# DLR-RB/QUEASARS

Hardware: AMD Instinct MI355X
Metric: circuit-evals/sec (EVQE population) at n qubits; achieved HBM GB/s vs roofline (higher is better)
Workload: dtype f64; 1 GPU; 20-qubit EVQE population=64 per GPU, 4 layers, random Ising Hamiltonian (210 terms), fp64 (BASELINE.json configs[1]); n_qubits=20, population_per_gpu=64, layers=4, pauli_terms=210, parallelism=1 GPU

## Files before the change

include/qsv.h:

```cpp
#ifndef QSV_H
#define QSV_H

#include <stddef.h>
#include <stdint.h>

#ifdef __cplusplus
extern "C" {
#endif

typedef struct qsv_handle qsv_t;

enum { QSV_OP_ID = 0, QSV_OP_U = 1, QSV_OP_CU3 = 2 };
enum { QSV_F64 = 0, QSV_F32 = 1 };
enum { QSV_NO_CONTROL = 0xFF };

enum {
    QSV_OK = 0,
    QSV_E_ARG = -1,
    QSV_E_DEVICE = -2,
    QSV_E_STATE = -3,
    QSV_E_UNSUPPORTED = -4
};

typedef struct qsv_op {
// ... 227 lines not shown
int qsv_adjoint_describe(int n_qubits, int n_ops, const qsv_op* ops, int n_params, int n_wrt, const int32_t* wrt, int capacity_runs,
                         uint64_t* out_masks, int32_t* out_first_op, int32_t* out_last_op, int64_t* out_n_gates,
                         int32_t* out_tile_bits, int32_t* out_low_bits);
int qsv_adjoint_gradient_circuits(qsv_t* h, int n_evals, const int* circuit_ids, const int64_t* param_offsets, const double* params,
                                  const int64_t* wrt_offsets , const int32_t* wrt,
                                  double* out , double* out_values );
int qsv_adjoint_gradient_device(qsv_t* h, int n_evals, const int* circuit_ids, int width, const double* device_values, void* ready_event,
                                const int64_t* wrt_offsets, const int32_t* wrt, int out_width, double* device_out,
                                double* device_out_values );
typedef struct qsv_adjoint_stats_t {
    int64_t n_gates;
    int64_t n_runs;
    int64_t n_state_sweeps;
    int64_t scratch_bytes;
    int64_t n_allocations;
} qsv_adjoint_stats_t;
int qsv_adjoint_stats(const qsv_t* h, qsv_adjoint_stats_t* out);


int qsv_observables_create(qsv_t* h, int n_observables, const int64_t* term_offsets, const uint64_t* x_mask,
                           const uint64_t* z_mask, const double* coeff_re, const double* coeff_im, int* out_set_id);
int qsv_observables_destroy(qsv_t* h, int set_id);
int qsv_eval_observables(qsv_t* h, int set_id, int n_evals, const int* circuit_ids, const int64_t* param_offsets,
                         const double* params, double* out);


#define QSV_TABLE_SENTINEL 0x7FF8C0DEC0DE0001ull
int qsv_fitness_table_wait(const volatile uint64_t* own, int count, volatile int64_t* done, int stride, int world, int rank,
                           int64_t step, int budget_us);


int qsv_set_option(qsv_t* h, const char* name, int value);

long long qsv_replayed_pushes(const qsv_t* h);

int qsv_set_profiling(qsv_t* h, int enabled);
int qsv_get_profile(const qsv_t* h, qsv_profile* out);

int qsv_bench_gate(qsv_t* h, int target, int control, double theta, double phi, double lambda, int reps,
                   double* out_ms_per_sweep);

int qsv_bench_ops(qsv_t* h, int n_ops, const qsv_op* ops, int reps, double* out_ms_per_rep, int* out_n_passes);

int qsv_plan_build(int n_qubits, int dtype, int n_ops, const qsv_op* ops, const qsv_plan_config* cfg,
                   uint32_t* out_words, size_t capacity_words, size_t* n_words);

int qsv_split_describe(int n_qubits, int n_ops, const qsv_op* ops, int max_side, uint64_t* mask_a, qsv_op* ops_a,
                       int capacity_a, int* n_ops_a, qsv_op* ops_b, int capacity_b, int* n_ops_b);

#define QSV_SPLIT_MAX_KEYS 8
int qsv_split_describe_reduced(int n_qubits, int n_ops, const qsv_op* ops, int max_side, uint64_t* mask_a, qsv_op* ops_a,
                               int capacity_a, int* n_ops_a, qsv_op* ops_b, int capacity_b, int* n_ops_b,
                               uint32_t* simulated_keys, uint32_t* final_keys, int* key_bits, int* qubits);

const char* qsv_version(void);

#ifdef __cplusplus
}
#endif
#endif
```

queasars_amd/_lib.py:

```python

from __future__ import annotations

import ctypes as C
import os
import threading
from pathlib import Path

import numpy as np

from queasars_amd import _build

QSV_OK, QSV_E_ARG, QSV_E_DEVICE, QSV_E_STATE, QSV_E_UNSUPPORTED = 0, -1, -2, -3, -4
QSV_F64, QSV_F32 = 0, 1


class QsvOp(C.Structure):
    _fields_ = [
        ("kind", C.c_uint8),
        ("target", C.c_uint8),
        ("control", C.c_uint8),
        ("flags", C.c_uint8),
        ("p_theta", C.c_int32),
        ("p_phi", C.c_int32),
        ("p_lambda", C.c_int32),
# ... 224 lines not shown
    "qsv_statevector": (C.c_int, [_P, C.c_int, _P, C.c_int, _P]),
    "qsv_probabilities": (C.c_int, [_P, C.c_int, _P, C.c_int, _P]),
    "qsv_sample": (C.c_int, [_P, C.c_int, _P, C.c_int, C.c_int, C.c_uint64, _P]),
    "qsv_sample_batch": (C.c_int, [_P, C.c_int, _P, _P, _P, C.c_int, C.c_uint64, _P, _P]),
    "qsv_sample_cvar_batch": (C.c_int, [_P, C.c_int, _P, _P, _P, C.c_int, C.c_uint64, C.c_double, _P]),
    "qsv_exact_cvar_batch": (C.c_int, [_P, C.c_int, _P, _P, _P, C.c_double, _P]),
    "qsv_top_states": (C.c_int, [_P, C.c_int, _P, _P, _P, C.c_int, _P, _P, _P]),
    "qsv_cvar_device": (C.c_int, [_P, C.c_int, _P, C.c_int, _P, _P, C.c_int, C.c_uint64, C.c_double, _P, C.c_int, _P]),
    "qsv_value_cache_create": (C.c_int, [_P, C.c_int, C.c_int, _P]),
    "qsv_value_cache_destroy": (C.c_int, [_P, C.c_int]),
    "qsv_value_cache_clear": (C.c_int, [_P, C.c_int]),
    "qsv_value_cache_stats": (C.c_int, [_P, C.c_int, _P]),
    "qsv_sample_lookup": (C.c_int, [_P, C.c_int, C.c_int, _P, _P, _P, C.c_int, C.c_uint64, _P, _P]),
    "qsv_sample_lookup_finish": (C.c_int, [_P, C.c_int, C.c_int64, _P, C.c_double, _P, _P]),
    "qsv_gradient_describe": (C.c_int, [C.c_int, _P, C.c_int, _P]),
    "qsv_gradient_circuits": (C.c_int, [_P, C.c_int, _P, _P, _P, _P, _P, _P, _P]),
    "qsv_gradient_device": (C.c_int, [_P, C.c_int, _P, C.c_int, _P, _P, _P, _P, C.c_int, _P, _P]),
    "qsv_gradient_stats": (C.c_int, [_P, C.POINTER(QsvGradientStats)]),
    "qsv_gradient_plan_create": (C.c_int, [_P, C.c_int, _P, C.c_int, _P, _P, C.c_int, C.POINTER(C.c_int), C.POINTER(C.c_int64)]),
    "qsv_gradient_plan_run": (C.c_int, [_P, C.c_int, _P, _P, _P]),
    "qsv_gradient_plan_destroy": (C.c_int, [_P, C.c_int]),
    "qsv_gradient_plan_stats": (C.c_int, [_P, C.c_int, C.POINTER(QsvGradientPlanStats)]),
    "qsv_adjoint_describe": (C.c_int, [C.c_int, C.c_int, _P, C.c_int, C.c_int, _P, C.c_int, _P, _P, _P, C.POINTER(C.c_int64),
                                       C.POINTER(C.c_int32), C.POINTER(C.c_int32)]),
    "qsv_adjoint_gradient_circuits": (C.c_int, [_P, C.c_int, _P, _P, _P, _P, _P, _P, _P]),
    "qsv_adjoint_gradient_device": (C.c_int, [_P, C.c_int, _P, C.c_int, _P, _P, _P, _P, C.c_int, _P, _P]),
    "qsv_adjoint_stats": (C.c_int, [_P, C.POINTER(QsvAdjointStats)]),
    "qsv_observables_create": (C.c_int, [_P, C.c_int, _P, _P, _P, _P, _P, C.POINTER(C.c_int)]),
    "qsv_observables_destroy": (C.c_int, [_P, C.c_int]),
    "qsv_eval_observables": (C.c_int, [_P, C.c_int, C.c_int, _P, _P, _P, _P]),
    "qsv_set_option": (C.c_int, [_P, C.c_char_p, C.c_int]),
    "qsv_fitness_table_wait": (C.c_int, [C.c_void_p, C.c_int, C.c_void_p, C.c_int, C.c_int, C.c_int, C.c_int64, C.c_int]),
    "qsv_replayed_pushes": (C.c_longlong, [_P]),
    "qsv_set_profiling": (C.c_int, [_P, C.c_int]),
    "qsv_get_profile": (C.c_int, [_P, C.POINTER(QsvProfile)]),
    "qsv_bench_gate": (C.c_int, [_P, C.c_int, C.c_int, C.c_double, C.c_double, C.c_double, C.c_int, C.POINTER(C.c_double)]),
    "qsv_bench_ops": (C.c_int, [_P, C.c_int, _P, C.c_int, C.POINTER(C.c_double), C.POINTER(C.c_int)]),
    "qsv_split_describe": (
        C.c_int,
        [C.c_int, C.c_int, _P, C.c_int, C.POINTER(C.c_uint64), _P, C.c_int, C.POINTER(C.c_int), _P, C.c_int, C.POINTER(C.c_int)],
    ),
    "qsv_split_describe_reduced": (
        C.c_int,
        [C.c_int, C.c_int, _P, C.c_int, C.POINTER(C.c_uint64), _P, C.c_int, C.POINTER(C.c_int), _P, C.c_int, C.POINTER(C.c_int),
         _P, _P, _P, _P],
    ),
    "qsv_plan_build": (
        C.c_int,
        [C.c_int, C.c_int, C.c_int, _P, C.POINTER(QsvPlanConfig), _P, C.c_size_t, C.POINTER(C.c_size_t)],
    ),
}

_lock = threading.Lock()
_lib = None


class QsvLibraryError(RuntimeError):
    """libqsv is missing or could not be loaded.  There is deliberately no fallback."""


def library_path() -> Path:
    override = os.environ.get("QSV_LIBRARY")
    return Path(override) if override else _build.LIB_PATH


def load(build_if_missing: bool = True) -> C.CDLL:
# ... 36 lines not shown
```

queasars_amd/csrc/kernels.hip:

```cpp
#include "kernels.hpp"
#include "plan.hpp"

#include <hip/hip_runtime.h>

#include <type_traits>
#include <utility>

namespace qsv {

template <typename real>
struct alignas(2 * sizeof(real)) cx {
    real re, im;
};

#if defined(__HIP_DEVICE_COMPILE__)
#define QSV_CONST_AS __attribute__((address_space(4)))
#else
#define QSV_CONST_AS
#endif
using cu32p = const QSV_CONST_AS uint32_t*;
using cf64p = const QSV_CONST_AS double*;
template <typename T>
__device__ __forceinline__ const QSV_CONST_AS T* as_constant(const T* p) {
    return (const QSV_CONST_AS T*)(p);
// ... 3095 lines not shown
            out[0 * 64 + pi] = acc_one[e];
            out[1 * 64 + pi] = acc_d[e];
#pragma unroll
            for (int q = 0; q < 6; ++q) out[(2 + q) * 64 + pi] = acc_low[e][q];
#pragma unroll
            for (uint32_t q = 0; q < 10; ++q) {
                double v = 0.0;
                if (q < uint32_t(HB) && q < lm) v = acc_high[e][q < uint32_t(HB) ? q : 0];
                if (q >= lm && (worker >> (q - lm) & 1u)) v = acc_one[e];
                out[(8 + q) * 64 + pi] = v;
            }
        }
    }
}

template <uint32_t J>
__device__ __forceinline__ double factor_pairing_unrolled(const double* a, const double* b) {
    constexpr uint32_t NQ = J * J;
    double t = 0.0;
#pragma unroll
    for (uint32_t j = 0; j < J; ++j) t = fma(a[j], b[j], t);
#pragma unroll
    for (uint32_t e = J; e < NQ; e += 2) t += 2.0 * fma(a[e], b[e], -a[e + 1] * b[e + 1]);
    return t;
}
__device__ __forceinline__ double factor_pairing(const double* a, const double* b, uint32_t n_keys) {
    switch (n_keys) {
        case 0: return factor_pairing_unrolled<1>(a, b);
        case 1: return factor_pairing_unrolled<2>(a, b);
        case 2: return factor_pairing_unrolled<4>(a, b);
        default: return factor_pairing_unrolled<8>(a, b);
    }
}

constexpr unsigned kFactorParts = 8;
constexpr uint32_t kFactorSlices = kFactorParts / 2;

constexpr uint32_t kFactorBigEntries = 1024;
constexpr uint32_t kFactorBigSlices = 8;
constexpr size_t kFactorBigFinal = size_t(2) * kFactorBigSlices * kFactorWeights * kFactorBigEntries;
constexpr size_t factor_big_slot_doubles_c() { return kFactorBigFinal + size_t(2) * kFactorWeights * kFactorBigEntries; }
size_t factor_big_slot_doubles() { return factor_big_slot_doubles_c(); }
constexpr uint32_t kFactorBigCounters = 8;
size_t factor_big_slot_counters() { return kFactorBigCounters; }

template <typename real, int J>
__device__ __forceinline__ void factor_moments_big_body(const EvalDesc& ev, const uint32_t* __restrict__ sp,
                                                        const cx<real>* __restrict__ sides, uint64_t side_stride,
                                                        const double* __restrict__ diag, const double* __restrict__ side_diag,
                                                        double* __restrict__ scratch, uint32_t* __restrict__ counters, cx<real>* stage, double* dstage) {
    constexpr uint32_t NQ = J * J, PITCH = J + 1, PER = uint32_t(J) * 64u / 256u;
    const bool swap = sp[3] & 1u;
    const uint32_t side = blockIdx.x & 1u, slice = (blockIdx.x >> 1) & (kFactorBigSlices - 1), group = blockIdx.x / (2 * kFactorBigSlices);
    if (group * 256u >= NQ) return;
    const uint32_t bits = sp[1 + side];
    const uint32_t own_d = sp[kSplitSideDiag + side];
    const bool in_place = own_d != kNoSideDiag;
    const uint32_t mask = sp[kSplitMaskX + side];
    diag = in_place ? side_diag + own_d : diag;
    const uint32_t tid = threadIdx.x;
    const cx<real>* ta = sides + uint64_t(ev.state_slot) * side_stride;
    const cx<real>* tab = ta + ((side == 0) == swap ? side_stride >> 1 : 0);
    const uint32_t pi = group * 256u + tid;
    uint32_t ja, jb, part;
    split_entry_of<J>(pi, &ja, &jb, &part);
    const uint32_t n_local = bits < 6u ? 1u << bits : 64u, n_blocks = bits < 6u ? 1u : 1u << (bits - 6u);
// ... 246 lines not shown
    } else if (tid == bx * by + 2) {
        v = -d00 * factor_pairing(gram[0], gram[1], n_keys);
    }
    const double total = block_sum_256(v, red);
    if (tid == 0) result_out[ev.out_index] = total;
}

struct ReducedRows {
    uint32_t x_block, entry;
    double sign;
};
__device__ __forceinline__ ReducedRows factor_reduced_rows(uint32_t reduced, uint32_t n_keys, uint32_t pi) {
    const uint32_t n_final = reduced & 3u, n_sim = (reduced >> 2) & 3u;
    uint32_t ja, jb, part;
    if (n_keys == 1)
        split_entry_of<2>(pi, &ja, &jb, &part);
    else if (n_keys == 2)
        split_entry_of<4>(pi, &ja, &jb, &part);
    else
        split_entry_of<8>(pi, &ja, &jb, &part);
    uint32_t ra = 0, rb = 0;
    for (uint32_t r = 0; r < n_keys; ++r) {
        const uint32_t key = reduced >> (4u + 2u * r) & 3u;
        ra |= (ja >> key & 1u) << r;
        rb |= (jb >> key & 1u) << r;
    }
    const uint32_t x_block = ra & ((1u << n_final) - 1u);
    if (x_block != (rb & ((1u << n_final) - 1u))) return ReducedRows{0u, 0u, 0.0};
    const uint32_t sa = ra >> n_final, sb = rb >> n_final, J = 1u << n_sim;
    uint32_t entry = sa;
    double sign = 1.0;
    if (sa != sb) {
        const uint32_t lo = sa < sb ? sa : sb, hi = sa < sb ? sb : sa;
        uint32_t o = hi - lo - 1u;
        for (uint32_t i = 0; i < lo; ++i) o += J - 1u - i;
        entry = J + 2u * o + (part - 1u);
        if (part == 2u && sa > sb) sign = -1.0;
    }
    return ReducedRows{x_block, entry, sign};
}
__device__ __forceinline__ uint64_t factor_reduced_positions(uint32_t slots0, uint32_t slots1, uint32_t bits) {
    uint64_t positions = 0;
    for (uint32_t p = 0; p < bits; ++p) {
        const uint32_t q = (p < 8u ? slots0 : slots1) >> (4u * (p & 7u)) & 15u;
        positions = (positions & ~(uint64_t(15) << (4u * q))) | uint64_t(p) << (4u * q);
    }
    return positions;
}
__device__ __forceinline__ double factor_reduced_value(const double* partial, const ReducedRows& rows, uint64_t positions, uint32_t reduced,
                                                       uint32_t bits, uint32_t waves_per_block, uint32_t w) {
    if (rows.sign == 0.0) return 0.0;
    const uint32_t low_bits = bits - (reduced & 3u), x_block = rows.x_block;
    uint32_t weight = w;
    if (w >= 2u) {
        const uint32_t at = uint32_t(positions >> (4u * (w - 2u))) & 15u;
        if (at < low_bits)
            weight = 2u + at;
        else if (x_block >> (at - low_bits) & 1u)
            weight = 0u;
        else
            return 0.0;
    }
    constexpr uint32_t kMostWaves = 4;
    const double* first = partial + (size_t(x_block * waves_per_block) * kFactorWeights + weight) * 64 + rows.entry;
    double part[kMostWaves][4];
#pragma unroll
    for (uint32_t g = 0; g < kMostWaves; ++g)
#pragma unroll
// ... 128 lines not shown
                const int32_t shift = int32_t(half_x * uint32_t(sizeof(cx<real>)));
                half_rows.at[j] = (j >> (n_keys - 1u)) == hh ? local : local + (hh ? -shift : shift);
            }
            half_rows.on = true;
            half_first = wave < kWaves ? blocks * hh + wave : 0xffffffu;
            half_end = blocks * (hh + 1u);
        }
        if (body_keys == 0)
#endif
            factor_side_body<real, 1, true>(tab, bits, mask, diag, half_first, step, stage, dstage_all + w * 64, sink, dq QSV_PSTAMP_ARGS,
                                            half_rows, half_end);
#ifndef QSV_ABL_TAIL_GRAM
        else if (body_keys == 1)
            factor_side_body<real, 2, true>(tab, bits, mask, diag, half_first, step, stage, dstage_all + w * 64, sink, dq QSV_PSTAMP_ARGS,
                                            half_rows, half_end);
        else if (body_keys == 2)
            factor_side_body<real, 4, false>(tab, bits, mask, diag, half_first, step, stage, dstage_all + w * 64, sink, dq QSV_PSTAMP_ARGS,
                                             half_rows, half_end);
        else if (halves) {
            const uint32_t mine_first = 4u * hh, x0 = hh << (kFusedLdsRowsBits - kFusedLdsRowsKeys - 1);
            auto row_of = [=](const cx<real>* base, uint32_t j, uint32_t) -> const cx<real>* {
                return (j >> 2) == (mine_first >> 2) ? base + (j & 3u) * uint32_t(kFusedLdsRowPitch)
                                                    : base + uint32_t(kFusedHalvesImport / sizeof(cx<real>)) + (j & 3u) * uint32_t(kFusedHalvesImportPitch) - x0;
            };
            factor_side_body_pairs<real, 2, true>(reinterpret_cast<const cx<real>*>(lds), bits, mask, diag, wave < kWaves ? kWaves * hh + wave : 0xffffffu, 2u * kWaves, stage,
                                                  dstage_all + w * 64, sink, dq_pairs QSV_PSTAMP_ARGS, row_of);
        } else if (table_lds_rows)
            factor_side_body_pairs<real, 2, true>(reinterpret_cast<const cx<real>*>(lds), bits, mask, diag, wave < kWaves ? wave : 0xffffffu, step, stage,
                                                  dstage_all + w * 64, sink, dq_pairs QSV_PSTAMP_ARGS);
        else
            factor_side_body_pairs<real, 2, false>(tab, bits, mask, diag, wave < kWaves ? wave : 0xffffffu, step, stage, dstage_all + w * 64, sink, dq_pairs QSV_PSTAMP_ARGS);
#endif
    }
    __syncthreads();
    QSV_PSTAMP(1);
#ifdef QSV_ABL_NO_HANDOFF
    return;
#endif
    double* slot = a.factor_scratch + size_t(ev.state_slot) * factor_slot_doubles();
    double* mine = slot + (size_t(xy) * kFactorSlices + hh) * kFactorWeights * 64;
    bool handed = false;
    if constexpr (REDUCED) {
        if (n_final) {
            const uint32_t pi = tid & (NQ - 1u);
            const ReducedRows rows = factor_reduced_rows(reduced, n_keys, pi);
            const uint64_t positions = factor_reduced_positions(sp[kSplitReducedSlots + 2u * xy], sp[kSplitReducedSlots + 2u * xy + 1u], bits);
            for (uint32_t idx = tid; idx < (2u + bits) * NQ; idx += blockDim.x) {
                const uint32_t w = idx >> (2u * n_keys);
                const double v = factor_reduced_value(partial, rows, positions, reduced, bits, waves_per_block, w);
                __hip_atomic_store(mine + w * 64 + pi, v, __ATOMIC_RELAXED, __HIP_MEMORY_SCOPE_AGENT);
            }
            handed = true;
        }
    }
    if (!handed)
        for (uint32_t idx = tid; idx < (2u + bits) * NQ; idx += blockDim.x) {
            const uint32_t w = idx / NQ, pi = idx % NQ;
            const double v = factor_sum_partials(partial, kWaves, w, pi, n_keys);
            __hip_atomic_store(mine + w * 64 + pi, v, __ATOMIC_RELAXED, __HIP_MEMORY_SCOPE_AGENT);
        }
    asm volatile("s_waitcnt vmcnt(0)" ::: "memory");
    __syncthreads();
    if (tid == 0) {
        const uint32_t add = halves ? 1u : 2u;
        const uint32_t before = __hip_atomic_fetch_add(a.factor_counters + size_t(kFactorCountersPerSlot) * ev.state_slot, add, __ATOMIC_RELAXED, __HIP_MEMORY_SCOPE_AGENT);
        *flag = ((before + add) & 3u) == 0u;
    }
    __syncthreads();
    QSV_PSTAMP(2);
    if (!*flag) return;
    const uint32_t bx = sp[1], by = sp[2];
    const uint32_t masks[2] = {sp[kSplitMaskX], sp[kSplitMaskY]};
    double coupling = 0.0;
    uint32_t qa_i = 0, qb_i = 0;
    if (tid < bx * by) {
        qa_i = tid / by;
        qb_i = tid % by;
        uint32_t qa = 0, qb = 0;
        for (uint32_t m = masks[0], k = 0; m; m &= m - 1, ++k)
            if (k == qa_i) qa = uint32_t(__builtin_ctz(m));
        for (uint32_t m = masks[1], k = 0; m; m &= m - 1, ++k)
            if (k == qb_i) qb = uint32_t(__builtin_ctz(m));
        coupling = a.quad[qa * a.n_full + qb];
    }
    const double d00 = whole_diag[0];
    double* gram = reinterpret_cast<double*>(lds);
    const uint32_t side_bits[2] = {bx, by};
    const bool any_halves = ev.flags & kEvalHalves;
    const bool two_halves[2] = {any_halves && (!REDUCED || sp[kSplitReduced] == 0u) && bx + n_keys == uint32_t(kFusedLdsRowsBits),
                                any_halves && (!REDUCED || sp[kSplitReduced + 1] == 0u) && by + n_keys == uint32_t(kFusedLdsRowsBits)};
    {
        constexpr uint32_t kMaxPerThread = (kFactorWeights * 64 + 255) / 256;
        double fetched[2][kMaxPerThread];
#pragma unroll
        for (uint32_t s2 = 0; s2 < 2; ++s2)
#pragma unroll
            for (uint32_t it = 0; it < kMaxPerThread; ++it) {
                const uint32_t idx = tid + it * blockDim.x;
                fetched[s2][it] = 0.0;
                if (idx < (2u + side_bits[s2]) * NQ) {
                    const double* entry = slot + size_t(s2) * kFactorSlices * kFactorWeights * 64 + (idx / NQ) * 64 + idx % NQ;
                    fetched[s2][it] = __hip_atomic_load(entry, __ATOMIC_RELAXED, __HIP_MEMORY_SCOPE_AGENT);
                    if (two_halves[s2])
                        fetched[s2][it] += __hip_atomic_load(entry + kFactorWeights * 64, __ATOMIC_RELAXED, __HIP_MEMORY_SCOPE_AGENT);
                }
            }
#pragma unroll
        for (uint32_t s2 = 0; s2 < 2; ++s2)
#pragma unroll
            for (uint32_t it = 0; it < kMaxPerThread; ++it) {
                const uint32_t idx = tid + it * blockDim.x;
                if (idx < (2u + side_bits[s2]) * NQ)
                    gram[size_t(s2) * kFactorWeights * kFactorPitch + (idx / NQ) * kFactorPitch + idx % NQ] = fetched[s2][it];
            }
    }
    __syncthreads();
    const double* g0 = gram;
    const double* g1 = gram + size_t(kFactorWeights) * kFactorPitch;
    double v = 0.0;
    if (tid < bx * by) {
        if (coupling != 0.0) v = 4.0 * coupling * factor_pairing(g0 + (2 + qa_i) * kFactorPitch, g1 + (2 + qb_i) * kFactorPitch, n_keys);
    } else if (tid == bx * by) {
        v = factor_pairing(g0 + kFactorPitch, g1, n_keys);
    } else if (tid == bx * by + 1) {
        v = factor_pairing(g0, g1 + kFactorPitch, n_keys);
    } else if (tid == bx * by + 2) {
        v = -d00 * factor_pairing(g0, g1, n_keys);
    }
    double* red = reinterpret_cast<double*>(flag) + 1;
#pragma unroll
    for (int off = 32; off > 0; off >>= 1) v += __shfl_xor(v, off);
    if ((tid & 63u) == 0 && wave < 4) red[wave] = v;
    __syncthreads();
    if (tid == 0) a.result_out[ev.out_index] = red[0] + red[1] + red[2] + red[3];
    QSV_PSTAMP(3);
}

hipError_t launch_factor(int dtype, unsigned n_evals, double* scratch, const double* quad, int n_qubits, hipStream_t stream,
                         const PassArgs& a, double* scratch_big, uint32_t* big_counters, int most_keys) {
    if (n_evals == 0) return hipSuccess;
    if (most_keys > 3 && (!scratch_big || !big_counters)) return hipErrorInvalidValue;
    const dim3 grid(most_keys >= 5 ? 2 * kFactorBigSlices * 4 : most_keys == 4 ? 2 * kFactorBigSlices : kFactorParts, n_evals);
    if (dtype == 0)
        hipLaunchKernelGGL(factor_moments_kernel<double>, grid, dim3(256), 0, stream, a.plan, a.evals,
                           static_cast<const cx<double>*>(a.wtab), a.wtab_stride, a.diag, scratch, scratch_big, big_counters, a.side_diag);
    else
        hipLaunchKernelGGL(factor_moments_kernel<float>, grid, dim3(256), 0, stream, a.plan, a.evals,
                           static_cast<const cx<float>*>(a.wtab), a.wtab_stride, a.diag, scratch, scratch_big, big_counters, a.side_diag);
    hipLaunchKernelGGL(factor_combine_kernel, dim3(n_evals), dim3(most_keys > 3 ? 1024 : 256), 0, stream, a.plan, a.evals, scratch,
                       scratch_big, quad, uint32_t(n_qubits), a.diag, a.result_out);
    return hipGetLastError();
}

__device__ __forceinline__ uint32_t extract_bits(uint32_t v, uint32_t mask) {
    uint32_t out = 0, pos = 0;
    while (mask) {
        const uint32_t low = mask & (0u - mask);
        if (v & low) out |= 1u << pos;
        ++pos;
        mask ^= low;
// ... 657 lines not shown
```

queasars_amd/csrc/kernels.hpp:

```cpp
#pragma once

#include <hip/hip_runtime.h>

#include <cstdint>

#include "../../include/qsv.h"

namespace qsv {

struct EvalDesc {
    uint32_t plan_base;
    uint32_t mat_base;
    uint32_t state_slot;
    uint32_t out_index;
    uint32_t param_base;
    uint32_t n_params;
    uint32_t flags;
    uint32_t split_base;
};
constexpr uint32_t kEvalSide = 1u, kEvalSideB = 2u, kEvalNull = 4u;
constexpr uint32_t kEvalFused = 8u;
constexpr uint32_t kEvalPrefix = 16u;
constexpr uint32_t kEvalHalves = 32u;
constexpr int kSideExtraBits = 4;
constexpr int kSideMaxOwnBits = 16;
constexpr uint32_t kNoSideDiag = 0xffffffffu;
constexpr uint32_t kSplitLoopCols = 4, kSplitLoopPos = 9, kSplitMaskX = 14, kSplitMaskY = 15, kSplitLaneTable = 16, kSplitWaveTable = 144,
                   kSplitChunkLow = 160, kSplitChunkHigh = 416, kSplitSideDiag = 672, kSplitReduced = 674, kSplitReducedSlots = 676,
                   kSplitBlockWords = 680;
constexpr int kSplitLoopBits = 5, kSplitMaxLoopX = 2;
constexpr uint32_t kSplitFlags = 3, kSplitSwapXY = 1u;

enum PassMode : uint32_t {
    kModeSynthFirst = 1u,
    kModeFinalStore = 2u,
    kModeFinalDiag = 4u,
    kModeDirectResult = 32u,
    kModeFinalProbs = 64u,
    kModeStreaming = 16u,
    kModeSidesOnly = 128u,
    kModeFusedFactor = 256u,
    kModeFusedLdsTable = 512u,
    kModeTileMajor = 1024u,
    kModeFusedPrepare = 8u,
    kModeMasked = 2048u,
    kModeSidePrepare = 4096u,
    kModeFusedReduced = 8192u,
};
struct ActiveMask {
    const uint8_t* flags = nullptr;
    uint32_t stride = 1;
};
#if defined(__HIPCC__)
__device__ __forceinline__ bool masked_out(const uint8_t* flags, uint32_t stride, uint32_t eval) {
    return flags != nullptr && flags[eval / stride] == 0;
}
#endif

struct PassArgs {
    const uint32_t* plan;
    const double* mats;
    const EvalDesc* evals;
    void* states;
    void* wtab;
    const double* diag;
    double* partials;
    uint64_t state_stride;
    uint64_t wtab_stride;
    uint32_t pass_index;
    uint32_t mode;
    uint32_t tiles_per_block;
    uint32_t region_stride;
    const EvalDesc* host_evals;
    EvalDesc* evals_out;
    const double* host_params;
    double* mats_out;
    double* result_out;
    uint32_t partial_chunks;
    const double* quad;
    double* factor_scratch;
    uint32_t* factor_counters;
// ... 166 lines not shown
```

queasars_amd/csrc/qsv_api.hip:

```cpp
#include <hip/hip_runtime.h>
#include <immintrin.h>

#include <algorithm>
#include <atomic>
#include <chrono>
#include <cmath>
#include <cstdio>
#include <condition_variable>
#include <cstring>
#include <functional>
#include <memory>
#include <mutex>
#include <string>
#include <thread>
#include <unordered_map>
#include <vector>

#include "../../include/qsv.h"
#include "adjoint.hpp"
#include "gradient.hpp"
#include "value_cache.hpp"
#include "kernels.hpp"
#include "plan.hpp"
#include "split.hpp"
// ... 184 lines not shown
    bool fused_factor = true;
    int split_max_keys = 5;
    bool quadratic = false;
    DeviceBuffer d_quad;
    DeviceBuffer d_fterms;
    uint32_t n_fterms = 0;
    DeviceBuffer d_fpart;
    DeviceBuffer d_factor;
    DeviceBuffer d_factor_count;
    DeviceBuffer d_factor_big;
    DeviceBuffer d_factor_big_count;
    uint32_t stream_mode = 0;
    mutable std::mutex mu;
    std::atomic<std::thread::id> batch_owner{};

    int n_terms = 0;
    bool diagonal = false;
    bool has_diag_part = false;
    int n_groups = 0;
    DeviceBuffer d_z, d_cre, d_diag, d_term_partials, d_groups, d_term_odd;
    DeviceBuffer d_order, d_sorted;
    bool order_valid = false;
    int pauli_nb = 0;

    std::unordered_map<int, Circuit> circuits;
    int next_circuit_id = 1;
    std::unordered_map<int, PrefixState> prefixes;
    int next_prefix_id = 1;
    DeviceBuffer d_prefix;
    DeviceBuffer d_sdiag;
    size_t sdiag_used = 0;
    bool side_diag = true;
    bool final_controls = true;
    bool sides_r3 = true;
    size_t prefix_slots = 0;
    std::vector<uint32_t> prefix_free;
    size_t prefix_used = 0;
    std::unordered_map<std::string, int> inline_cache;
    std::unordered_map<int, ObservableSet> obs_sets;
    int next_obs_id = 1;
    DeviceBuffer d_obs_partials, d_obs_values;
    std::unique_ptr<WorkerPool> pool;
    std::mutex pool_mu;

    struct CoalesceRequest {
        int circuit_id = 0;
        const double* params = nullptr;
        int n_params = 0;
        double value = 0.0;
        int rc = QSV_OK;
        std::string err;
        bool done = false;
    };
    std::mutex cq_mu;
    std::condition_variable cq_cv;
    std::vector<CoalesceRequest*> cq;
    std::atomic<size_t> cq_count{0};
    bool cq_collecting = false;
    size_t cq_expected = 0;
    uint64_t cq_batches = 0;

    DeviceBuffer d_arena;
    size_t arena_used_words = 0;
    DeviceBuffer d_states;
    DeviceBuffer d_wtab;
    uint64_t wtab_stride = 0;
// ... 1114 lines not shown
        auto launch_sides = [&](size_t lo, size_t hi, uint32_t extra_mode, int r) -> int {
            int threads, passes;
            size_t lds;
            unsigned tiles;
            shape_of(lo, hi, &threads, &lds, &passes, &tiles);
            if (extra_mode & kModeFusedFactor) threads = at_least_four_waves(threads);
            bool any_halves = false, any_reduced = false;
            if (extra_mode & kModeFusedFactor)
                for (size_t i = lo; i < hi; ++i) {
                    const Circuit& c = *circs[eval_of(first + i)];
                    any_halves |= side_form(h, c).halves;
                    any_reduced |= &side_form(h, c) == &c.reduced;
                }
            a.tiles_per_block = (extra_mode & kModeFusedFactor) ? tiles : 1u;
            const unsigned grid_x = (extra_mode & kModeFusedFactor) ? (any_halves ? 2u : 1u) : tiles;
            a.evals = batch_evals(h) + first + lo;
            a.host_evals = descs_base(h) + first + lo;
            a.evals_out = static_cast<EvalDesc*>(h->d_batch.ptr) + first + lo;
            for (int p = 0; p < passes; ++p) {
                a.pass_index = uint32_t(p);
                a.mode = ((p == 0 ? (mode | kModeFusedPrepare | extra_mode) : mode) & ~uint32_t(kModeSidesOnly)) | h->stream_mode;
                const int kind = p == 0 ? 0 : 1;
                size_t need = lds;
                if (p == 0) need = std::max(need, kFusedPrepareLdsBytes);
                if (p == 0 && (extra_mode & kModeFusedFactor)) need = std::max(need, kFusedFactorLdsBytes);
                size_t working = 0;
                for (size_t i = lo; i < hi; ++i) working += working_workgroups(side_form(h, *circs[eval_of(first + i)]));
                if (p == 0 && (extra_mode & kModeFusedFactor) && h->dtype == QSV_F64 && (h->fused_lds_table || any_halves) && working <= size_t(h->n_cus)) {
                    a.mode |= kModeFusedLdsTable;
                    need = std::max(need, kFusedLdsTableEnd);
                }
                if (p == 0 && (extra_mode & kModeFusedFactor) && h->side_prepare) a.mode |= kModeSidePrepare;
                if (p == 0 && any_reduced) a.mode |= kModeFusedReduced;
                if (h->stamping) QSV_HIP(h, stamp(h, h->batch.launch_events[kind], true));
                QSV_LAUNCH(h, launch_pass(h->dtype, r, h->cfg.xmode, dim3(grid_x, unsigned(hi - lo), 2), threads, need, ws(h), a));
                record_pass(h, r, dim3(grid_x, unsigned(hi - lo), 2), threads, need, a);
                if (h->stamping) QSV_HIP(h, stamp(h, h->batch.launch_events[kind], false));
                h->prof.n_pass_launches += 1;
                h->prof.kernel_launches[kind] += 1;
            }
            return QSV_OK;
        };
        int rc2;
        hipStream_t const lane_of_group = h->work;
        if (two_chains) h->work = chain_st;
        auto launch_sides_by_r = [&](size_t lo, size_t hi, uint32_t extra_mode) -> int {
            for (size_t at = lo; at < hi;) {
                const int r = side_form(h, *circs[eval_of(first + at)]).side_r == 3 ? 3 : h->geo.r;
                size_t end = at;
                bool halves_here = false;
                while (end < hi && (side_form(h, *circs[eval_of(first + end)]).side_r == 3 ? 3 : h->geo.r) == r) {
                    halves_here |= side_form(h, *circs[eval_of(first + end)]).halves;
                    ++end;
                }
                for (size_t from = at; from < end;) {
                    size_t to = end;
                    if (halves_here && (extra_mode & kModeFusedFactor)) {
                        size_t wg = 0;
                        for (to = from; to < end && wg + working_workgroups(side_form(h, *circs[eval_of(first + to)])) <= size_t(h->n_cus); ++to)
                            wg += working_workgroups(side_form(h, *circs[eval_of(first + to)]));
                        if (to == from) to = from + 1;
                    }
                    const int rc3 = launch_sides(from, to, extra_mode, r);
                    if (rc3) return rc3;
                    from = to;
                }
// ... 959 lines not shown
        const size_t budget = size_t(2) << 30;
        group = int(std::max<size_t>(1, std::min<size_t>(256, budget / state_bytes)));
    }
    h->group = group;
    {
        const uint64_t tiles_per_launch = uint64_t(geo.blocks_per_state) * uint64_t(group);
        h->tiles_per_block = (tiles_per_launch >= 4096 && geo.blocks_per_state >= 2) ? 2 : 1;
    }
    h->tiles_per_block_later = h->tiles_per_block;
    if (const char* env = getenv("QSV_TILES_PER_BLOCK")) h->tiles_per_block = h->tiles_per_block_later = std::max(1, atoi(env));
    if (const char* env = getenv("QSV_TILES_PER_BLOCK_LATER")) h->tiles_per_block_later = std::max(1, atoi(env));
    auto bail = [&](hipError_t err, const char* what) {
        std::string msg = std::string(what) + ": " + hipGetErrorString(err);
        qsv_destroy(h);
        return fail(nullptr, QSV_E_DEVICE, msg);
    };
    if ((e = hipStreamCreateWithFlags(&h->stream, hipStreamNonBlocking)) != hipSuccess) return bail(e, "hipStreamCreate");
    h->own_stream = true;
    if (const char* env = getenv("QSV_SPLIT")) h->split_enabled = atoi(env) != 0;
    if (const char* env = getenv("QSV_SPLIT_SAMPLE")) h->split_sampling = atoi(env) != 0;
    if (const char* env = getenv("QSV_FACTOR")) h->factor_enabled = atoi(env) != 0;
    if (getenv("QSV_NO_FUSED_FACTOR")) h->fused_factor = false;
    if (const char* env = getenv("QSV_CHAIN_STREAM")) h->chain_enabled = atoi(env) != 0;
    if (const char* env = getenv("QSV_POLL")) h->poll_results = atoi(env) != 0;
    if (const char* env = getenv("QSV_REPEAT")) h->repeat_enabled = atoi(env) != 0;
    if (const char* env = getenv("QSV_REPLAY")) h->replay_enabled = atoi(env) != 0;
    if (const char* env = getenv("QSV_HOST_TIMING")) h->timing.on = atoi(env) != 0;
    if (const char* env = getenv("QSV_REPEAT_DESCS")) h->repeat_device_descs = atoi(env) != 0;
    if (const char* env = getenv("QSV_FUSED_LDS")) h->fused_lds_table = atoi(env) != 0;
    if (const char* env = getenv("QSV_SIDE_PREPARE")) h->side_prepare = atoi(env) != 0;
    if (const char* env = getenv("QSV_SIDE_DIAG")) h->side_diag = atoi(env) != 0;
    if (const char* env = getenv("QSV_SIDES_R3")) h->sides_r3 = atoi(env) != 0;
    if (const char* env = getenv("QSV_FINAL_CONTROLS")) h->final_controls = atoi(env) != 0;
    {
        int cus = 0;
        if (hipDeviceGetAttribute(&cus, hipDeviceAttributeMultiprocessorCount, device) == hipSuccess && cus > 0) h->n_cus = cus;
        int grid_y = 0;
        if (hipDeviceGetAttribute(&grid_y, hipDeviceAttributeMaxGridDimY, device) == hipSuccess && grid_y > 0)
            h->max_grid_y = h->device_max_grid_y = grid_y;
    }
    {
        int large_bar = 0;
        if (hipDeviceGetAttribute(&large_bar, hipDeviceAttributeIsLargeBar, device) != hipSuccess) large_bar = 0;
        h->bar_ship = false;
        if (const char* env = getenv("QSV_BAR")) h->bar_ship = large_bar != 0 && atoi(env) != 0;
    }
    if (const char* env = getenv("QSV_SPLIT_MAX_KEYS")) h->split_max_keys = std::max(0, std::min(kMaxSplitKeys, atoi(env)));
    h->stream_mode = state_bytes > (size_t(256) << 20) ? uint32_t(kModeStreaming) : 0u;
    if (const char* env = getenv("QSV_STREAMING")) h->stream_mode = atoi(env) ? uint32_t(kModeStreaming) : 0u;
    if (const char* env = getenv("QSV_STREAMS")) h->n_streams = std::max(1, std::min(4, atoi(env)));
    for (int i = 1; i < std::max(2, h->n_streams); ++i) {
        hipStream_t st = nullptr;
        if ((e = hipStreamCreateWithFlags(&st, hipStreamNonBlocking)) != hipSuccess) return bail(e, "hipStreamCreate");
        h->side_streams.push_back(st);
    }
    h->n_lane_streams = int(h->side_streams.size());
    if ((e = hipEventCreateWithFlags(&h->ev_join, hipEventDisableTiming)) != hipSuccess) return bail(e, "hipEventCreate");
    if ((e = hipMalloc(&h->d_states.ptr, state_bytes * size_t(group))) != hipSuccess) return bail(e, "hipMalloc(states)");
    h->d_states.bytes = state_bytes * size_t(group);
    h->wtab_stride = std::min<uint64_t>(uint64_t(1) << n_qubits, uint64_t(1) << (geo.k + int(kMaxCompactBits)));
    if ((e = hipMalloc(&h->d_wtab.ptr, size_t(h->wtab_stride) * h->amp_bytes * size_t(group))) != hipSuccess)
        return bail(e, "hipMalloc(compact tables)");
    h->d_wtab.bytes = size_t(h->wtab_stride) * h->amp_bytes * size_t(group);
    if (h->split_enabled && n_qubits > geo.k && n_qubits <= 28) {
        h->side_stride = uint64_t(2) << (geo.k + kSideExtraBits);
        h->side_slots = 256;
// ... 2253 lines not shown
    std::lock_guard<std::mutex> lock(h->mu);
    h->epoch += 1;
    const std::string key(name);
    if (key == "split") {
        if (value != 0 && !h->d_side.ptr && h->n > h->geo.k && h->n <= 28)
            return fail(h, QSV_E_ARG, "this handle was created without side tables (QSV_SPLIT=0): splitting cannot be switched on");
        h->split_enabled = value != 0;
    } else if (key == "factor") {
        if (value != 0 && h->split_enabled && h->d_side.ptr && !h->d_factor.ptr)
            return fail(h, QSV_E_ARG, "this handle was created without the factorised path (QSV_FACTOR=0)");
        h->factor_enabled = value != 0;
    } else if (key == "fused_factor") {
        h->fused_factor = value != 0;
    } else if (key == "chain_stream") {
        h->chain_enabled = value != 0;
    } else if (key == "poll_results") {
        h->poll_results = value != 0;
    } else if (key == "repeat_layout") {
        h->repeat_enabled = value != 0;
    } else if (key == "replay_launches") {
        h->replay_enabled = value != 0;
    } else if (key == "split_max_keys") {
        if (value < 0 || value > kMaxSplitKeys) return fail(h, QSV_E_ARG, "split_max_keys must be between 0 and 5");
        h->split_max_keys = value;
    } else if (key == "split_sampling") {
        h->split_sampling = value != 0;
    } else if (key == "fused_lds_table") {
        h->fused_lds_table = value != 0;
    } else if (key == "side_prepare") {
        h->side_prepare = value != 0;
    } else if (key == "final_controls") {
        h->final_controls = value != 0;
        h->epoch += 1;
    } else if (key == "sides_r3") {
        h->sides_r3 = value != 0;
    } else if (key == "side_diag") {
        if (h->side_diag != (value != 0)) {
            QSV_HIP(h, sync_streams(h));
            for (auto& kv : h->circuits) kv.second.uploaded = false;
            h->sdiag_used = 0;
        }
        h->side_diag = value != 0;
    } else if (key == "streams") {
        if (value < 1 || value > h->n_lane_streams + 1) return fail(h, QSV_E_ARG, "streams must be between 1 and the number the handle was created with");
        h->n_streams = value;
    } else if (key == "max_grid_y") {
        if (value < 0 || value > h->device_max_grid_y) return fail(h, QSV_E_ARG, "max_grid_y must be between 0 and the device's largest gridDim.y");
        h->max_grid_y = value ? value : h->device_max_grid_y;
    } else if (key == "gradient_chunk") {
        if (value < 0 || value > (1 << 20)) return fail(h, QSV_E_ARG, "gradient_chunk must be between 0 and 1048576");
        h->grad_chunk = value ? value : kGradientChunkRows;
    } else {
        return fail(h, QSV_E_ARG, "unknown option '" + key + "'");
    }
    return QSV_OK;
}

int qsv_set_profiling(qsv_t* h, int enabled) {
    if (!h) return QSV_E_ARG;
    std::lock_guard<std::mutex> lock(h->mu);
    h->epoch += 1;
    h->profiling = enabled != 0;
    return QSV_OK;
}

long long qsv_replayed_pushes(const qsv_t* h) {
    if (!h) return QSV_E_ARG;
    std::lock_guard<std::mutex> lock(h->mu);
    return (long long)h->replayed_pushes;
}

int qsv_get_profile(const qsv_t* h, qsv_profile* out) {
    if (!h || !out) return QSV_E_ARG;
    std::lock_guard<std::mutex> lock(h->mu);
    *out = h->prof;
    return QSV_OK;
}

static int bench_ops_locked(qsv_t* h, int n_ops, const qsv_op* ops, int reps, double* out_ms_per_rep,
                            int* out_n_passes) {
    if (!out_ms_per_rep || reps < 1) return fail(h, QSV_E_ARG, "bad arguments");
    QSV_HIP(h, hipSetDevice(h->device));
    int id = 0;
    int rc = register_circuit(h, n_ops, ops, 0, &id, false);
    if (rc) return rc;
    Circuit& c = h->circuits.find(id)->second;
    auto cleanup = [&]() { h->circuits.erase(id); };
    std::vector<Circuit*> cc{&c};
    if ((rc = batch_layout(h, cc, std::vector<int64_t>{0})) || (rc = batch_ship(h, 0, 1, kNoValues))) {
        h->batch.circs.clear();
        cleanup();
        return rc;
    }
    h->batch.circs.clear();
    PassArgs a{};
    a.plan = static_cast<const uint32_t*>(h->d_arena.ptr);
// ... 157 lines not shown
```

Measured before the change: 1.604 million circuit-evals/s.

## Hand off and pair only live Gram entries in fused reduced factor kernel

In the fused reduced-factor path with three keys, the kernel now works out which of the 64 packed Gram entries can be nonzero for the current key mask. It compacts those lanes with ballot, mbcnt and ds_permute. Only those entries are stored to the handoff slot, fetched back and paired, using a specialised unrolled pairing function. A closed-form offset also replaces a small loop. The aim is to cut cross-block atomic traffic and pairing arithmetic, at the price of extra wave shuffles and more complex indexing.

```diff
diff --git a/include/qsv.h b/include/qsv.h
--- a/include/qsv.h
+++ b/include/qsv.h
@@ -283,6 +283,8 @@
 
 int qsv_set_option(qsv_t* h, const char* name, int value);
 
+int qsv_live_entries(int n_keys, unsigned key_mask, int* out_pi);
+
 long long qsv_replayed_pushes(const qsv_t* h);
 
 int qsv_set_profiling(qsv_t* h, int enabled);
diff --git a/queasars_amd/_lib.py b/queasars_amd/_lib.py
--- a/queasars_amd/_lib.py
+++ b/queasars_amd/_lib.py
@@ -280,6 +280,7 @@
     "qsv_set_option": (C.c_int, [_P, C.c_char_p, C.c_int]),
     "qsv_fitness_table_wait": (C.c_int, [C.c_void_p, C.c_int, C.c_void_p, C.c_int, C.c_int, C.c_int, C.c_int64, C.c_int]),
     "qsv_replayed_pushes": (C.c_longlong, [_P]),
+    "qsv_live_entries": (C.c_int, [C.c_int, C.c_uint, C.POINTER(C.c_int)]),
     "qsv_set_profiling": (C.c_int, [_P, C.c_int]),
     "qsv_get_profile": (C.c_int, [_P, C.POINTER(QsvProfile)]),
     "qsv_bench_gate": (C.c_int, [_P, C.c_int, C.c_int, C.c_double, C.c_double, C.c_double, C.c_int, C.POINTER(C.c_double)]),
diff --git a/queasars_amd/csrc/kernels.hip b/queasars_amd/csrc/kernels.hip
--- a/queasars_amd/csrc/kernels.hip
+++ b/queasars_amd/csrc/kernels.hip
@@ -3151,6 +3151,15 @@
         default: return factor_pairing_unrolled<8>(a, b);
     }
 }
+template <uint32_t L>
+__device__ __forceinline__ double factor_pairing_live(const double* a, const double* b) {
+    double t = 0.0;
+#pragma unroll
+    for (uint32_t j = 0; j < 8; ++j) t = fma(a[j], b[j], t);
+#pragma unroll
+    for (uint32_t e = 8; e < L; e += 2) t += 2.0 * fma(a[e], b[e], -a[e + 1] * b[e + 1]);
+    return t;
+}
 
 constexpr unsigned kFactorParts = 8;
 constexpr uint32_t kFactorSlices = kFactorParts / 2;
@@ -3463,8 +3472,7 @@
     double sign = 1.0;
     if (sa != sb) {
         const uint32_t lo = sa < sb ? sa : sb, hi = sa < sb ? sb : sa;
-        uint32_t o = hi - lo - 1u;
-        for (uint32_t i = 0; i < lo; ++i) o += J - 1u - i;
+        const uint32_t o = hi - lo - 1u + lo * (2u * J - 1u - lo) / 2u;
         entry = J + 2u * o + (part - 1u);
         if (part == 2u && sa > sb) sign = -1.0;
     }
@@ -3659,6 +3667,20 @@
             factor_side_body_pairs<real, 2, false>(tab, bits, mask, diag, wave < kWaves ? wave : 0xffffffu, step, stage, dstage_all + w * 64, sink, dq_pairs QSV_PSTAMP_ARGS);
 #endif
     }
+    uint32_t live_log = 6u, live_pi = 0u;
+    if constexpr (REDUCED) {
+        const uint32_t key_mask = n_keys == 3u && (a.mode & kModeFusedLive) ? live_key_mask(sp[kSplitReduced], sp[kSplitReduced + 1]) : 0u;
+        if (key_mask) {
+            const uint32_t lane = tid & 63u;
+            const bool live = live_entry(key_mask, lane, nullptr);
+            const uint64_t live_lanes = __ballot(live);
+            const uint32_t below = __builtin_amdgcn_mbcnt_hi(uint32_t(live_lanes >> 32), __builtin_amdgcn_mbcnt_lo(uint32_t(live_lanes), 0u));
+            live_log = 6u - uint32_t(__builtin_popcount(key_mask));
+            const uint32_t to = live ? below : (1u << live_log) + (lane - below);
+            const uint32_t ranked = uint32_t(__builtin_amdgcn_ds_permute(int(to << 2), int(lane)));
+            live_pi = uint32_t(__builtin_amdgcn_ds_bpermute(int((lane & ((1u << live_log) - 1u)) << 2), int(ranked)));
+        }
+    }
     __syncthreads();
     QSV_PSTAMP(1);
 #ifdef QSV_ABL_NO_HANDOFF
@@ -3669,13 +3691,22 @@
     bool handed = false;
     if constexpr (REDUCED) {
         if (n_final) {
-            const uint32_t pi = tid & (NQ - 1u);
-            const ReducedRows rows = factor_reduced_rows(reduced, n_keys, pi);
+            const bool live_only = live_log < 6u;
+            const uint32_t at_log = live_only ? live_log : 2u * n_keys, at = tid & ((1u << at_log) - 1u);
+            const ReducedRows rows = factor_reduced_rows(reduced, n_keys, live_only ? live_pi : at);
             const uint64_t positions = factor_reduced_positions(sp[kSplitReducedSlots + 2u * xy], sp[kSplitReducedSlots + 2u * xy + 1u], bits);
-            for (uint32_t idx = tid; idx < (2u + bits) * NQ; idx += blockDim.x) {
-                const uint32_t w = idx >> (2u * n_keys);
+            for (uint32_t idx = tid; idx < (2u + bits) << at_log; idx += blockDim.x) {
+                const uint32_t w = idx >> at_log;
                 const double v = factor_reduced_value(partial, rows, positions, reduced, bits, waves_per_block, w);
-                __hip_atomic_store(mine + w * 64 + pi, v, __ATOMIC_RELAXED, __HIP_MEMORY_SCOPE_AGENT);
+                __hip_atomic_store(mine + w * 64 + at, v, __ATOMIC_RELAXED, __HIP_MEMORY_SCOPE_AGENT);
+            }
+            handed = true;
+        } else if (live_log < 6u) {
+            const uint32_t at = tid & ((1u << live_log) - 1u), pi = live_pi;
+            for (uint32_t idx = tid; idx < (2u + bits) << live_log; idx += blockDim.x) {
+                const uint32_t w = idx >> live_log;
+                const double v = factor_sum_partials(partial, kWaves, w, pi, n_keys);
+                __hip_atomic_store(mine + w * 64 + at, v, __ATOMIC_RELAXED, __HIP_MEMORY_SCOPE_AGENT);
             }
             handed = true;
         }
@@ -3719,14 +3750,15 @@
     {
         constexpr uint32_t kMaxPerThread = (kFactorWeights * 64 + 255) / 256;
         double fetched[2][kMaxPerThread];
+        const uint32_t per_weight = REDUCED ? 1u << (live_log < 6u ? live_log : 2u * n_keys) : 1u << (2 * n_keys);
 #pragma unroll
         for (uint32_t s2 = 0; s2 < 2; ++s2)
 #pragma unroll
             for (uint32_t it = 0; it < kMaxPerThread; ++it) {
                 const uint32_t idx = tid + it * blockDim.x;
                 fetched[s2][it] = 0.0;
-                if (idx < (2u + side_bits[s2]) * NQ) {
-                    const double* entry = slot + size_t(s2) * kFactorSlices * kFactorWeights * 64 + (idx / NQ) * 64 + idx % NQ;
+                if (idx < (2u + side_bits[s2]) * per_weight) {
+                    const double* entry = slot + size_t(s2) * kFactorSlices * kFactorWeights * 64 + (idx / per_weight) * 64 + idx % per_weight;
                     fetched[s2][it] = __hip_atomic_load(entry, __ATOMIC_RELAXED, __HIP_MEMORY_SCOPE_AGENT);
                     if (two_halves[s2])
                         fetched[s2][it] += __hip_atomic_load(entry + kFactorWeights * 64, __ATOMIC_RELAXED, __HIP_MEMORY_SCOPE_AGENT);
@@ -3737,22 +3769,52 @@
 #pragma unroll
             for (uint32_t it = 0; it < kMaxPerThread; ++it) {
                 const uint32_t idx = tid + it * blockDim.x;
-                if (idx < (2u + side_bits[s2]) * NQ)
-                    gram[size_t(s2) * kFactorWeights * kFactorPitch + (idx / NQ) * kFactorPitch + idx % NQ] = fetched[s2][it];
+                if (idx < (2u + side_bits[s2]) * per_weight)
+                    gram[size_t(s2) * kFactorWeights * kFactorPitch + (idx / per_weight) * kFactorPitch + idx % per_weight] = fetched[s2][it];
             }
     }
     __syncthreads();
     const double* g0 = gram;
     const double* g1 = gram + size_t(kFactorWeights) * kFactorPitch;
     double v = 0.0;
-    if (tid < bx * by) {
-        if (coupling != 0.0) v = 4.0 * coupling * factor_pairing(g0 + (2 + qa_i) * kFactorPitch, g1 + (2 + qb_i) * kFactorPitch, n_keys);
-    } else if (tid == bx * by) {
-        v = factor_pairing(g0 + kFactorPitch, g1, n_keys);
-    } else if (tid == bx * by + 1) {
-        v = factor_pairing(g0, g1 + kFactorPitch, n_keys);
-    } else if (tid == bx * by + 2) {
-        v = -d00 * factor_pairing(g0, g1, n_keys);
+    bool paired = false;
+    if constexpr (REDUCED) {
+        if (live_log < 6u) {
+            const double* pa = g0;
+            const double* pb = g1;
+            double scale = 1.0;
+            bool term = true;
+            if (tid < bx * by) {
+                term = coupling != 0.0;
+                pa = g0 + (2 + qa_i) * kFactorPitch;
+                pb = g1 + (2 + qb_i) * kFactorPitch;
+                scale = 4.0 * coupling;
+            } else if (tid == bx * by) {
+                pa = g0 + kFactorPitch;
+            } else if (tid == bx * by + 1) {
+                pb = g1 + kFactorPitch;
+            } else if (tid == bx * by + 2) {
+                scale = -d00;
+            } else {
+                term = false;
+            }
+            if (term) {
+                const double t = live_log == 5u ? factor_pairing_live<32>(pa, pb) : live_log == 4u ? factor_pairing_live<16>(pa, pb) : factor_pairing_live<8>(pa, pb);
+                v = scale * t;
+            }
+            paired = true;
+        }
+    }
+    if (!paired) {
+        if (tid < bx * by) {
+            if (coupling != 0.0) v = 4.0 * coupling * factor_pairing(g0 + (2 + qa_i) * kFactorPitch, g1 + (2 + qb_i) * kFactorPitch, n_keys);
+        } else if (tid == bx * by) {
+            v = factor_pairing(g0 + kFactorPitch, g1, n_keys);
+        } else if (tid == bx * by + 1) {
+            v = factor_pairing(g0, g1 + kFactorPitch, n_keys);
+        } else if (tid == bx * by + 2) {
+            v = -d00 * factor_pairing(g0, g1, n_keys);
+        }
     }
     double* red = reinterpret_cast<double*>(flag) + 1;
 #pragma unroll
diff --git a/queasars_amd/csrc/kernels.hpp b/queasars_amd/csrc/kernels.hpp
--- a/queasars_amd/csrc/kernels.hpp
+++ b/queasars_amd/csrc/kernels.hpp
@@ -46,7 +46,39 @@
     kModeMasked = 2048u,
     kModeSidePrepare = 4096u,
     kModeFusedReduced = 8192u,
-};
+    kModeFusedLive = 16384u,
+};
+inline __host__ __device__ void live_entry_rows(uint32_t pi, uint32_t* ja_out, uint32_t* jb_out) {
+    uint32_t ja = pi, jb = pi;
+    if (pi >= 8u) {
+        const uint32_t o = (pi - 8u) >> 1;
+        ja = (o >= 7u) + (o >= 13u) + (o >= 18u) + (o >= 22u) + (o >= 25u) + (o >= 27u);
+        jb = ja + 1u + o - ja * (15u - ja) / 2u;
+    }
+    *ja_out = ja;
+    *jb_out = jb;
+}
+inline __host__ __device__ bool live_entry(uint32_t key_mask, uint32_t pi, uint32_t* rank_out) {
+    uint32_t ja, jb;
+    live_entry_rows(pi, &ja, &jb);
+    if (rank_out) {
+        uint32_t rank = 0;
+        for (uint32_t below = 0; below < pi; ++below) {
+            uint32_t a, b;
+            live_entry_rows(below, &a, &b);
+            rank += ((a ^ b) & key_mask) == 0u ? 1u : 0u;
+        }
+        *rank_out = rank;
+    }
+    return ((ja ^ jb) & key_mask) == 0u;
+}
+inline __host__ __device__ uint32_t live_key_mask(uint32_t reduced_x, uint32_t reduced_y) {
+    auto of_side = [](uint32_t word) {
+        const uint32_t n_final = word & 3u;
+        return (n_final > 0u ? 1u << (word >> 4 & 3u) : 0u) | (n_final > 1u ? 1u << (word >> 6 & 3u) : 0u) | (n_final > 2u ? 1u << (word >> 8 & 3u) : 0u);
+    };
+    return of_side(reduced_x) | of_side(reduced_y);
+}
 struct ActiveMask {
     const uint8_t* flags = nullptr;
     uint32_t stride = 1;
diff --git a/queasars_amd/csrc/qsv_api.hip b/queasars_amd/csrc/qsv_api.hip
--- a/queasars_amd/csrc/qsv_api.hip
+++ b/queasars_amd/csrc/qsv_api.hip
@@ -240,6 +240,7 @@
     size_t sdiag_used = 0;
     bool side_diag = true;
     bool final_controls = true;
+    bool live_entries = true;
     bool sides_r3 = true;
     size_t prefix_slots = 0;
     std::vector<uint32_t> prefix_free;
@@ -1420,6 +1421,7 @@
                 }
                 if (p == 0 && (extra_mode & kModeFusedFactor) && h->side_prepare) a.mode |= kModeSidePrepare;
                 if (p == 0 && any_reduced) a.mode |= kModeFusedReduced;
+                if (p == 0 && any_reduced && h->live_entries) a.mode |= kModeFusedLive;
                 if (h->stamping) QSV_HIP(h, stamp(h, h->batch.launch_events[kind], true));
                 QSV_LAUNCH(h, launch_pass(h->dtype, r, h->cfg.xmode, dim3(grid_x, unsigned(hi - lo), 2), threads, need, ws(h), a));
                 record_pass(h, r, dim3(grid_x, unsigned(hi - lo), 2), threads, need, a);
@@ -2445,6 +2447,7 @@
     if (const char* env = getenv("QSV_SIDE_DIAG")) h->side_diag = atoi(env) != 0;
     if (const char* env = getenv("QSV_SIDES_R3")) h->sides_r3 = atoi(env) != 0;
     if (const char* env = getenv("QSV_FINAL_CONTROLS")) h->final_controls = atoi(env) != 0;
+    if (const char* env = getenv("QSV_LIVE_ENTRIES")) h->live_entries = atoi(env) != 0;
     {
         int cus = 0;
         if (hipDeviceGetAttribute(&cus, hipDeviceAttributeMultiprocessorCount, device) == hipSuccess && cus > 0) h->n_cus = cus;
@@ -4764,6 +4767,8 @@
     } else if (key == "final_controls") {
         h->final_controls = value != 0;
         h->epoch += 1;
+    } else if (key == "live_entries") {
+        h->live_entries = value != 0;
     } else if (key == "sides_r3") {
         h->sides_r3 = value != 0;
     } else if (key == "side_diag") {
@@ -4794,6 +4799,19 @@
     h->epoch += 1;
     h->profiling = enabled != 0;
     return QSV_OK;
+}
+
+int qsv_live_entries(int n_keys, unsigned key_mask, int* out_pi) {
+    if (n_keys != 3 || key_mask > 7u || !out_pi) return QSV_E_ARG;
+    for (int i = 0; i < 64; ++i) out_pi[i] = -1;
+    int count = 0;
+    for (uint32_t pi = 0; pi < 64; ++pi) {
+        uint32_t rank = 0;
+        if (!live_entry(key_mask, pi, &rank)) continue;
+        out_pi[rank] = int(pi);
+        ++count;
+    }
+    return count;
 }
 
 long long qsv_replayed_pushes(const qsv_t* h) {
```

Measured after the change: 1.712 million circuit-evals/s (median of 6 runs). 6.8% higher.
